# stoneMo/DeepAVFusion

Hardware: AMD Instinct MI355X
Metric: AV-pairs/sec, DeepAVFusion ViT-B pre-training step (224px + 10s audio, image mask 0.75) (higher is better)
Workload: dtype bf16; 1 GPU; AVMAE(DeepAVFusion base) fwd+bwd+allreduce+AdamW, B=64/GPU, 224x224 RGB + (128,640) log-mel, masks 0.75/0.8, fusion attn_ratio 0.25 mlp_ratio 1.0; global_batch=64, parallelism=dp1, graph=True

## Files before the change

### deepavfusion_amd/csrc/gemm_tn_gang.h

```cpp
#pragma once

__device__ __attribute__((aligned(256))) unsigned short g_tng_zeros[128];

struct TGDesc { int prob; int bnbk; };
struct TGHeader {
  int head[8];
  int q_start[9];
  int pad[15];
};
static_assert(sizeof(TGHeader) == 128, "TGHeader layout");

constexpr int TG_WCH = 28;
constexpr int TG_WIT = 72;
struct TGItem { int prob, desc_first, r0c0, nrnc; };
struct TGWrite {
  char* ws;
  int prob_first, prob_count, item_count, count_total, write_header;
  int q_start[9];
  TNParams prob[TG_WCH];
  TGItem item[TG_WIT];
};
static_assert(sizeof(TGWrite) <= 4096, "kernel argument block");

__global__ __launch_bounds__(64) void gemm_tn_gang_write_kernel(const TGWrite w) {
  TGHeader* hd = reinterpret_cast<TGHeader*>(w.ws);
  TNParams* probs = reinterpret_cast<TNParams*>(w.ws + sizeof(TGHeader));
  TGDesc* desc = reinterpret_cast<TGDesc*>(w.ws + sizeof(TGHeader) + (size_t)w.count_total * sizeof(TNParams));
  const int b = blockIdx.x, t = threadIdx.x;
  if (b < w.item_count) {
    const TGItem it = w.item[b];
    const int nr = it.nrnc >> 16, nc = it.nrnc & 0xffff, r0 = it.r0c0 >> 16, c0 = it.r0c0 & 0xffff;
    for (int i = t; i < nr * nc; i += 64) desc[it.desc_first + i] = TGDesc{it.prob, ((r0 + i / nc) << 16) | (c0 + i % nc)};
    return;
  }
  const int* src = reinterpret_cast<const int*>(w.prob);
  int* dst = reinterpret_cast<int*>(probs + w.prob_first);
  for (int i = t; i < w.prob_count * (int)(sizeof(TNParams) / 4); i += 64) dst[i] = src[i];
  if (w.write_header) {
    if (t < 8) hd->head[t] = 0;
    if (t < 9) hd->q_start[t] = w.q_start[t];
  }
}

__device__ __forceinline__ uint32_t tng_magic(int rpb) { return rpb > 1 ? (uint32_t)(0x100000000ull / (uint32_t)rpb) : rpb == 1 ? 0xffffffffu : 0u; }
__device__ __forceinline__ long tng_row(int m, const RowMap& r, uint32_t magic) {
  if (r.rpb <= 0) return (long)m;
  int q = (int)__umulhi((uint32_t)m, magic);
  int rem = m - q * r.rpb;
  if (rem >= r.rpb) { rem -= r.rpb; ++q; }
  return (long)q * r.bs + r.off + rem;
}

template <int V> struct TGI { static constexpr int value = V; };
template <int OFF>
__device__ __forceinline__ bf16x8 tng_tr(uint32_t base) {
  static_assert(OFF >= 0 && OFF + 1024 < 65536, "ds offset field");
  union { s16x4 h2[2]; bf16x8 v; } u;
  asm volatile("ds_read_b64_tr_b16 %0, %2 offset:%3\n\tds_read_b64_tr_b16 %1, %2 offset:%4"
               : "=&v"(u.h2[0]), "=&v"(u.h2[1]) : "v"(base), "i"(OFF), "i"(OFF + 1024));
  return u.v;
}

__device__ __forceinline__ void tng_tile(const TNParams& p, const int bn, const int bk, const int dbg) {
  extern __shared__ __attribute__((aligned(16))) char smem[];
  const int tid = threadIdx.x, lane = tid & 63;
  const int wave = __builtin_amdgcn_readfirstlane(tid >> 6);
  const int wr = wave >> 2, wc = wave & 3;
  const int n0 = bn << 8, k0 = bk << 8;
  const int nk = (p.Mc + 63) >> 6;
  const int kend = (nk + 1) & ~1;
  const uint32_t amagic = tng_magic(p.amap.rpb), bmagic = tng_magic(p.bmap.rpb);

  int a_col[2], b_col[2], krow[2];
#pragma unroll
  for (int ee = 0; ee < 2; ++ee) krow[ee] = (wave * 2 + ee) * 4 + (lane >> 4);
#pragma unroll
  for (int h = 0; h < 2; ++h) {
    const int c16 = lane & 15;
    const int g = (c16 >> 1) ^ (2 * ((lane >> 4) & 3));
    int ac = n0 + h * 128 + g * 16 + (c16 & 1) * 8; ac = ac < p.N ? ac : p.N - 8;
    int bc = k0 + h * 128 + g * 16 + (c16 & 1) * 8; bc = bc < p.K ? bc : p.K - 8;
    a_col[h] = ac; b_col[h] = bc;
  }
  auto issue = [&](bool isA, int h, int d, int kt) {
    char* slot = smem + (isA ? 0 : NT256_BREG) + d * 32768 + h * NT256_HT + wave * 2048;
    const bool pad = kt >= nk;
    const int ktc = pad ? nk - 1 : kt;
#pragma unroll
    for (int ee = 0; ee < 2; ++ee) {
      const int m0 = ktc * 64 + krow[ee];
      const int m = m0 < p.Mc ? m0 : p.Mc - 1;
      const bf16_t* src;
      if (isA) src = (pad || m0 >= p.Mc) ? reinterpret_cast<const bf16_t*>(g_tng_zeros) + (lane & 15) * 8 : p.A + tng_row(m, p.amap, amagic) * p.lda + a_col[h];
      else src = p.B + tng_row(m, p.bmap, bmagic) * p.ldb + b_col[h];
      __builtin_amdgcn_global_load_lds(GLB_PTR(void, src), LDS_PTR(void, slot + ee * 1024), 16, 0, 0);
    }
// ... 95 lines not shown
      TNG_G0(0, 1, t + 1) TNG_G0(1, 1, t + 1) TNG_G0(2, 1, t + 1) TNG_G0(3, 1, t + 1)
    }
#undef TNG_G0
  } else {
#define TNG_G1(I, D, T)                                                              \
    {                                                                                \
      if ((I) == 0) { read_a(TGI<(D) * 32768>{}); read_b(b0, TGI<(D) * 32768>{}); }                              \
      if ((I) == 1) read_b(b1, TGI<(D) * 32768 + 16384>{});                                              \
      if ((I) == 2) read_a(TGI<(D) * 32768 + 16384>{});                                                  \
      TNG_SB;                                                                        \
      issue_for(I, D, T);                                                            \
      asm volatile("s_waitcnt lgkmcnt(0)" ::: "memory");                             \
      TNG_SB;                                                                        \
      if ((I) == 0) bias_acc(0);                                                     \
      if ((I) == 2) bias_acc(1);                                                     \
      __builtin_amdgcn_s_setprio(1);                                                 \
      mfmas((I) >> 1, ((I) == 1 || (I) == 2) ? 1 : 0);                              \
      __builtin_amdgcn_s_setprio(0);                                                 \
      TNG_SB;                                                                        \
      wait_vmcnt<6>();                                                               \
      TNG_SB;                                                                        \
      __builtin_amdgcn_s_barrier();                                                  \
      TNG_SB;                                                                        \
    }
    for (int t = 0; t < kend; t += 2) {
      TNG_G1(0, 0, t) TNG_G1(1, 0, t) TNG_G1(2, 0, t) TNG_G1(3, 0, t)
      TNG_G1(0, 1, t + 1) TNG_G1(1, 1, t + 1) TNG_G1(2, 1, t + 1) TNG_G1(3, 1, t + 1)
    }
#undef TNG_G1
  }
#undef TNG_SB
  asm volatile("s_waitcnt vmcnt(0)" ::: "memory");
  __builtin_amdgcn_s_barrier();

  if (dbg & 2) return;
  typedef __attribute__((address_space(1))) f32x4 gf4_t;
  __attribute__((address_space(1))) float* const Cg = (__attribute__((address_space(1))) float*)p.C;
#pragma unroll
  for (int qm = 0; qm < 2; ++qm)
#pragma unroll
    for (int rf = 0; rf < 2; ++rf) {
      const int n = n0 + qm * 128 + wr * 64 + rf * 32 + (lane & 31);
      const long rowoff = (long)(n < p.N ? n : p.N - 1) * p.ldc;
      f32x4 v[2][4];
#pragma unroll
      for (int qn = 0; qn < 2; ++qn)
#pragma unroll
        for (int g = 0; g < 4; ++g) {
          const f32x16& q = acc[qm][qn][rf];
          v[qn][g] = f32x4{q[4 * g + 0], q[4 * g + 1], q[4 * g + 2], q[4 * g + 3]};
        }
      if (p.beta) {
        f32x4 old[2][4];
#pragma unroll
        for (int qn = 0; qn < 2; ++qn)
#pragma unroll
          for (int g = 0; g < 4; ++g) {
            const int k = k0 + qn * 128 + wc * 32 + 8 * g + 4 * hi;
            old[qn][g] = *(const gf4_t*)(Cg + rowoff + (k < p.K ? k : p.K - 4));
          }
#pragma unroll
        for (int qn = 0; qn < 2; ++qn)
#pragma unroll
          for (int g = 0; g < 4; ++g) v[qn][g] += old[qn][g];
      }
#pragma unroll
      for (int qn = 0; qn < 2; ++qn)
#pragma unroll
        for (int g = 0; g < 4; ++g) {
          const int k = k0 + qn * 128 + wc * 32 + 8 * g + 4 * hi;
          if (n < p.N && k < p.K) *(gf4_t*)(Cg + rowoff + k) = v[qn][g];
        }
    }
  if (do_bias) {
#pragma unroll
    for (int qm = 0; qm < 2; ++qm)
#pragma unroll
      for (int rf = 0; rf < 2; ++rf) {
        const float tot = accb[qm][rf] + __shfl_xor(accb[qm][rf], 32, 64);
        const int n = n0 + qm * 128 + wr * 64 + rf * 32 + (lane & 31);
        if (hi == 0 && n < p.N) unsafeAtomicAdd(p.bias_grad + n, tot);
      }
  }
}

constexpr size_t TNG_LDS = NT256_LDS + 16;

__global__ __launch_bounds__(512) void gemm_tn_gang_kernel(char* __restrict__ ws, const int count, const int dbg) {
  extern __shared__ __attribute__((aligned(16))) char smem[];
  TGHeader* hd = reinterpret_cast<TGHeader*>(ws);
  const int* probs = reinterpret_cast<const int*>(ws + sizeof(TGHeader));
  const TGDesc* desc = reinterpret_cast<const TGDesc*>(ws + sizeof(TGHeader) + (size_t)count * sizeof(TNParams));
  volatile __attribute__((address_space(3))) int* slot = (volatile __attribute__((address_space(3))) int*)(smem + NT256_LDS);
  int xcd;
  asm volatile("s_getreg_b32 %0, hwreg(HW_REG_XCC_ID)" : "=s"(xcd));
  xcd &= 7;
  if (dbg & 8) xcd = blockIdx.x & 7;
  if (dbg & 16) xcd = (blockIdx.x >> 5) & 7;
  for (int a = 0; a < 8; ++a) {
    const int q = (xcd + a) & 7;
    const int qs = hd->q_start[q], qn = hd->q_start[q + 1] - qs;
    while (true) {
      if (threadIdx.x == 0) {
        const int t = __hip_atomic_load(&hd->head[q], __ATOMIC_RELAXED, __HIP_MEMORY_SCOPE_AGENT) >= qn
                          ? qn : __hip_atomic_fetch_add(&hd->head[q], 1, __ATOMIC_RELAXED, __HIP_MEMORY_SCOPE_AGENT);
        *slot = t;
      }
      __syncthreads();
      const int t = __builtin_amdgcn_readfirstlane(*slot);
      __syncthreads();
      if (t >= qn) break;
      const TGDesc d = desc[qs + t];
      const int pi = __builtin_amdgcn_readfirstlane(d.prob), bnbk = __builtin_amdgcn_readfirstlane(d.bnbk);
      union { TNParams p; int w[sizeof(TNParams) / 4]; } u;
#pragma unroll
      for (int i = 0; i < (int)(sizeof(TNParams) / 4); ++i) u.w[i] = __builtin_amdgcn_readfirstlane(probs[pi * (int)(sizeof(TNParams) / 4) + i]);
      tng_tile(u.p, bnbk >> 16, bnbk & 0xffff, dbg);
    }
  }
}
```

### deepavfusion_amd/_lib.py

```python
from __future__ import annotations

import ctypes as C
import os

import torch

_HERE = os.path.dirname(os.path.abspath(__file__))
LIB_PATH = os.path.join(_HERE, 'libdavfusion_hip.so')

_p, _i, _l, _f, _sz = C.c_void_p, C.c_int, C.c_long, C.c_float, C.c_size_t

ABI_VERSION = 9

SIGNATURES = {
    'dav_abi_version': [],
    'dav_build_flags': [],
    'dav_last_error_string': [],
    'dav_tune': [_i, _i],
    'dav_gemm_nt_bf16': [_p, _p, _i, _i, _i, _i, _i, _p, _p, _i, _p, _i, _p, _i, _p, _p, _p, _i, _i, _p, _p, _i, _i, _i, _f, _i, _p],
    'dav_gemm_nt_ln_bf16': [_p, _p, _i, _i, _i, _i, _i, _p, _p, _i, _p, _i, _p, _i, _p, _p, _p, _i, _i, _p, _p, _i, _i, _i, _f, _i, _p, _p],
    'dav_ln_fold_grouped': [_p, _i, _p],
    'dav_rowstats_cast': [_p, _l, _i, _i, _i, _p, _p, _p],
    'dav_layernorm_bwd_twin': [_p, _l, _p, _i, _p, _l, _p, _i, _i, _i, _f, _p, _p, _p, _p,
                               _p, _l, _i, _p, _l, _p, _l,
                               _p, _l, _i, _p, _l, _p, _l,
                               _p, _p, _p, _p, _sz, _p],
    'dav_nt_issue_log': [_i, _p, _i],
    'dav_nt_tune_set': [_p, _i],
    'dav_gemm_tn_bf16': [_p, _p, _i, _i, _i, _i, _i, _p, _p, _p, _i, _i, _p, _i, _p],
    'dav_gemm_tn_grouped_bf16': [_p, _i, _p],
    'dav_gemm_tn_gang_workspace_bytes': [_p, _i],
    'dav_gemm_tn_gang_bf16': [_p, _i, _p, _sz, _p],
    'dav_attn_fwd': [_p, _p, _p, _p, _p, _i, _i, _i, _i, _i, _i, _l, _i, _l, _i, _l, _i, _l, _i, _f, _p],
    'dav_attn_bwd': [_p] * 10 + [_i] * 6 + [_l, _i] * 8 + [_f, _p],
    'dav_attn_bwd_part': [_p] * 10 + [_i] * 6 + [_l, _i] * 8 + [_f, _i, _p],
    'dav_add_cast': [_p, _p, _p, _p, _l, _p],
    'dav_attn_bwd_ctx': [_p] * 10 + [_i] * 6 + [_l, _i] * 8 + [_f, _i, _i, _p],
    'dav_attn_bias_fwd': [_p, _p, _p, _p, _p, _i, _i, _i, _i, _i, _i, _l, _i, _l, _i, _l, _i, _l, _i, _f, _p, _i, _i, _p],
    'dav_attn_bias_bwd': [_p] * 10 + [_i] * 6 + [_l, _i] * 8 + [_f, _p, _i, _i, _p, _i, _p],
    'dav_attn_drop_fwd': [_p, _p, _p, _p, _p, _i, _i, _i, _i, _i, _i, _l, _i, _l, _i, _l, _i, _l, _i, _f, _p, _i, _f, _p],
    'dav_attn_drop_bwd': [_p] * 10 + [_i] * 6 + [_l, _i] * 8 + [_f, _p, _i, _f, _i, _i, _p],
    'dav_window_unfold': [_p, _i, _p, _i, _i, _i, _i, _i, _i, _f, _p, _i, _p],
    'dav_window_fold': [_p, _p, _p, _i, _i, _i, _i, _i, _i, _f, _p, _p],
    'dav_relpos_bias_build': [_p, _p, _p, _i, _i, _i, _i, _i, _f, _p, _p],
    'dav_relpos_bias_bwd': [_p, _p, _i, _i, _i, _i, _i, _i, _p, _p],
    'dav_layernorm_fwd': [_p, _l, _i, _p, _l, _i, _i, _i, _p, _p, _f, _p, _p, _p, _p, _p],
    'dav_layernorm_bwd': [_p, _l, _i, _p, _l, _i, _i, _i, _p, _p, _p, _p, _p,
                          _p, _l, _i, _p, _l, _p, _l,
                          _p, _l, _i, _p, _l, _p, _l,
                          _p, _p, _p, _sz, _p],
    'dav_layernorm_bwd_workspace_bytes': [_i, _i],
    'dav_layernorm_bwd_reduce_grouped': [_p, _i, _p],
    'dav_mask_build': [_p, _i, _i, _i, _p, _p, _p, _p, _p, _p],
    'dav_patch_gather': [_p, _i, _i, _i, _i, _p, _i, _p, _p],
    'dav_patch_gather3d': [_p, _i, _i, _i, _i, _i, _i, _p, _i, _p, _p],
    'dav_unshuffle_fwd': [_p, _p, _p, _p, _i, _i, _i, _i, _p, _l, _i, _p],
    'dav_rows_gather_cast': [_p, _l, _i, _p, _i, _i, _i, _p, _p],
    'dav_rows_axpy': [_p, _p, _p, _i, _i, _i, _p, _p],
    'dav_rows_scale_cast': [_p, _p, _i, _i, _i, _p, _p],
    'dav_dropout_rows': [_p, _i, _p, _p, _f, _p, _i, _i, _i, _p, _i, _p],
    'dav_unshuffle_bwd_reduce': [_p, _l, _i, _p, _i, _i, _i, _i, _p, _p, _p],
    'dav_patch_mse_fwd': [_p, _p, _p, _i, _i, _i, _i, _i, _p, _p, _p, _p, _p, _p],
    'dav_patch_mse_bwd': [_p, _p, _p, _p, _p, _p, _p, _i, _i, _i, _i, _p, _p],
    'dav_pair_expand': [_p, _p, _i, _i, _i, _i, _p, _p],
    'dav_pair_reduce': [_p, _i, _i, _i, _i, _p, _p, _p],
# ... 121 lines not shown
```

### deepavfusion_amd/csrc/gemm.hip

```cpp
#include <algorithm>
#include <array>
#include <atomic>
#include <cstdlib>
#include <map>
#include <mutex>
#include <vector>

#include "common.h"
#include "dav_kernels.h"

namespace {

struct RowMap {
  int rpb, bs, off;
};
__device__ __forceinline__ long map_row(int m, const RowMap& r) {
  return r.rpb > 0 ? (long)(m / r.rpb) * r.bs + r.off + (m % r.rpb) : (long)m;
}

struct NTParams {
  const bf16_t* A; const bf16_t* B;
  int M, N, K, lda, ldb;
  RowMap amap;
  const float* bias;
// ... 2039 lines not shown
    total_tiles += (long)((q.N + 127) / 128) * ((q.K + 127) / 128);
  }
  int first = 0;
  for (int i = 0; i < count; ++i) {
    const DavTnProblem& q = probs[i];
    TNParams& p = g.prob[i];
    p.A = (const bf16_t*)q.A; p.B = (const bf16_t*)q.B; p.Mc = q.Mc; p.N = q.N; p.K = q.K; p.lda = q.lda; p.ldb = q.ldb;
    p.amap = RowMap{q.a_rowmap[0], q.a_rowmap[1], q.a_rowmap[2]};
    p.bmap = RowMap{q.b_rowmap[0], q.b_rowmap[1], q.b_rowmap[2]};
    static const int tn_debug = getenv("DAV_TN_DEBUG") ? atoi(getenv("DAV_TN_DEBUG")) & 6 : 0;
    p.C = q.C; p.ldc = q.ldc; p.beta = (q.flags & 1) ? 0 : 1; p.bias_grad = q.bias_grad; p.debug_plain_store = tn_debug;
    const int tiles = ((q.N + 127) / 128) * ((q.K + 127) / 128), steps = q.Mc >> 6;
    int splits = (int)((1024 + total_tiles - 1) / total_tiles);
    const int max_splits = steps / 8 > 0 ? steps / 8 : 1;
    if (splits > max_splits) splits = max_splits;
    if (q.flags & 1) splits = 1;
    p.splits = splits;
    g.first_block[i] = first;
    first += tiles * splits;
  }
  g.first_block[count] = first;
  g.count = count | TN_XCD_RUNS;
  const TNGroup gl = g;
  DAV_LAUNCH((gemm_tn_grouped_kernel<128, 4, 2>), dim3(first), dim3(512), (size_t)2 * 2 * 64 * 128 * 2, stream, gl);
  return dav_launch_status();
}

extern "C" int dav_gemm_tn_grouped_bf16(const DavTnProblem* probs, int count, hipStream_t stream) {
  if (!probs) return DAV_ERR_SHAPE;
  return tn_grouped_impl(probs, count, stream);
}

namespace {
struct TGPlanItem { int prob, r0, c0, nr, nc; long weight; int queue, first; };
long tn_gang_plan(const DavTnProblem* probs, int count, std::vector<TGPlanItem>& items, int q_start[9]) {
  items.clear();
  for (int i = 0; i < count; ++i) {
    const DavTnProblem& q = probs[i];
    const int tn = (q.N + 255) / 256, tk = (q.K + 255) / 256;
    int nr = tn, nc = tk;
    while (nr * nc > 32) { if (nr >= nc) nr = (nr + 1) / 2; else nc = (nc + 1) / 2; }
    for (int r0 = 0; r0 < tn; r0 += nr)
      for (int c0 = 0; c0 < tk; c0 += nc) {
        const int r = std::min(nr, tn - r0), c = std::min(nc, tk - c0);
        items.push_back(TGPlanItem{i, r0, c0, r, c, (long)r * c * ((q.Mc + 127) / 128), 0, 0});
      }
  }
  std::vector<int> order(items.size());
  for (size_t i = 0; i < order.size(); ++i) order[i] = (int)i;
  std::stable_sort(order.begin(), order.end(), [&](int a, int b) { return probs[items[a].prob].Mc > probs[items[b].prob].Mc; });
  long load[8] = {0, 0, 0, 0, 0, 0, 0, 0};
  int tiles_q[8] = {0, 0, 0, 0, 0, 0, 0, 0};
  for (int oi : order) {
    int best = 0;
    for (int q = 1; q < 8; ++q) if (load[q] < load[best]) best = q;
    items[oi].queue = best; items[oi].first = tiles_q[best];
    load[best] += items[oi].weight; tiles_q[best] += items[oi].nr * items[oi].nc;
  }
  q_start[0] = 0;
  for (int q = 0; q < 8; ++q) q_start[q + 1] = q_start[q] + tiles_q[q];
  return q_start[8];
}
int tn_gang_check(const DavTnProblem* probs, int count) {
  if (count <= 0 || count > 4096) return DAV_ERR_SHAPE;
  for (int i = 0; i < count; ++i) {
    const DavTnProblem& q = probs[i];
    if (q.Mc <= 0 || q.N <= 0 || q.K <= 0 || (q.N & 7) || (q.K & 7) || (q.lda & 7) || (q.ldb & 7)) return DAV_ERR_SHAPE;
    if (q.N > (32767 << 8) || q.K > (32767 << 8) || (q.flags & ~1)) return DAV_ERR_SHAPE;
    if (((uintptr_t)q.A | (uintptr_t)q.B | (uintptr_t)q.C) & 15 || (q.ldc & 3)) return DAV_ERR_ALIGN;
  }
  return DAV_OK;
}
}

extern "C" size_t dav_gemm_tn_gang_workspace_bytes(const DavTnProblem* probs, int count) {
  if (!probs || tn_gang_check(probs, count) != DAV_OK) return 0;
  long tiles = 0;
  for (int i = 0; i < count; ++i) tiles += (long)((probs[i].N + 255) / 256) * ((probs[i].K + 255) / 256);
  return sizeof(TGHeader) + (size_t)count * sizeof(TNParams) + (size_t)tiles * sizeof(TGDesc);
}

extern "C" int dav_gemm_tn_gang_bf16(const DavTnProblem* probs, int count, void* workspace, size_t workspace_bytes, hipStream_t stream) {
  if (!probs || !workspace) return DAV_ERR_SHAPE;
  const int chk = tn_gang_check(probs, count);
  if (chk != DAV_OK) return chk;
  if ((uintptr_t)workspace & 15) return DAV_ERR_ALIGN;
  if (workspace_bytes < dav_gemm_tn_gang_workspace_bytes(probs, count)) return DAV_ERR_WORKSPACE;
  std::vector<TGPlanItem> items;
  int q_start[9];
  tn_gang_plan(probs, count, items, q_start);
#ifdef DAV_EXPERIMENTAL
  static const int dbg = getenv("DAV_TN_GANG_DEBUG") ? atoi(getenv("DAV_TN_GANG_DEBUG")) & 30 : 0;
#else
  static const int dbg = getenv("DAV_TN_GANG_DEBUG") ? atoi(getenv("DAV_TN_GANG_DEBUG")) & 24 : 0;
#endif
  bool header = true;
  std::vector<std::vector<const TGPlanItem*>> by_prob(count);
  for (const TGPlanItem& it : items) by_prob[it.prob].push_back(&it);
  TGWrite w;
  auto reset = [&](int first) {
    w.ws = (char*)workspace; w.prob_first = first; w.prob_count = 0; w.item_count = 0; w.count_total = count; w.write_header = 0;
    for (int q = 0; q < 9; ++q) w.q_start[q] = q_start[q];
  };
  auto flush = [&]() {
    if (!w.prob_count && !w.item_count && !header) return;
    w.write_header = header ? 1 : 0; header = false;
    const TGWrite wl = w;
    DAV_LAUNCH(gemm_tn_gang_write_kernel, dim3(wl.item_count + 1), dim3(64), 0, stream, wl);
  };
  reset(0);
  for (int i = 0; i < count; ++i) {
    if (w.prob_count == TG_WCH) { flush(); reset(i); }
    const DavTnProblem& q = probs[i];
    TNParams& p = w.prob[w.prob_count++];
    p.A = (const bf16_t*)q.A; p.B = (const bf16_t*)q.B; p.Mc = q.Mc; p.N = q.N; p.K = q.K; p.lda = q.lda; p.ldb = q.ldb;
    p.amap = RowMap{q.a_rowmap[0], q.a_rowmap[1], q.a_rowmap[2]};
    p.bmap = RowMap{q.b_rowmap[0], q.b_rowmap[1], q.b_rowmap[2]};
    p.C = q.C; p.ldc = q.ldc; p.beta = (q.flags & 1) ? 0 : 1; p.bias_grad = q.bias_grad; p.debug_plain_store = 0; p.splits = 1;
    for (const TGPlanItem* it : by_prob[i]) {
      if (w.item_count == TG_WIT) { flush(); reset(i + 1); }
      w.item[w.item_count++] = TGItem{i, q_start[it->queue] + it->first, (it->r0 << 16) | it->c0, (it->nr << 16) | it->nc};
    }
  }
  flush();
  static std::mutex dev_mu;
  static int dev_cus[64] = {0};
  int n_wg = 256;
  {
    int dev = 0;
    if (hipGetDevice(&dev) != hipSuccess || dev < 0 || dev >= 64) return DAV_ERR_HIP;
    std::lock_guard<std::mutex> lk(dev_mu);
    if (!dev_cus[dev]) {
      if (hipFuncSetAttribute((const void*)gemm_tn_gang_kernel, hipFuncAttributeMaxDynamicSharedMemorySize, 160 * 1024) != hipSuccess) return DAV_ERR_HIP;
      int cus = 256;
      (void)hipDeviceGetAttribute(&cus, hipDeviceAttributeMultiprocessorCount, dev);
      dev_cus[dev] = cus > 0 ? cus : 256;
    }
    n_wg = dev_cus[dev];
  }
  const long tiles = q_start[8];
  const int grid = (int)std::min<long>(n_wg, tiles);
  DAV_LAUNCH(gemm_tn_gang_kernel, dim3(grid), dim3(512), TNG_LDS, stream, (char*)workspace, count, dbg);
  return dav_launch_status();
}

extern "C" int dav_gemm_tn_bf16(const void* A, const void* B, int Mc, int N, int K, int lda, int ldb,
                                const int* a_rowmap, const int* b_rowmap, float* C, int ldc, int beta,
                                float* bias_grad, int variant, hipStream_t stream) {
  if (Mc <= 0 || N <= 0 || K <= 0 || (N & 7) || (K & 7) || (lda & 7) || (ldb & 7)) return DAV_ERR_SHAPE;
  if (((uintptr_t)A | (uintptr_t)B) & 15) return DAV_ERR_ALIGN;
  TNParams p;
  p.A = (const bf16_t*)A; p.B = (const bf16_t*)B; p.Mc = Mc; p.N = N; p.K = K; p.lda = lda; p.ldb = ldb;
  p.amap = mk(a_rowmap); p.bmap = mk(b_rowmap); p.C = C; p.ldc = ldc; p.beta = beta; p.bias_grad = bias_grad;
  p.debug_plain_store = (variant >> 8) & 1;
  variant &= ~256;
  const int steps = (Mc + 63) / 64;
  const int cfg = variant >> 4;
  if (!(variant & 15) && (Mc & 63) == 0 && (beta || cfg) && !(ldc & 3) && !((uintptr_t)C & 15)) {
    const int t128 = ((N + 127) / 128) * ((K + 127) / 128), t64 = ((N + 63) / 64) * ((K + 63) / 64);
    const bool big = cfg ? cfg == 1 : (Mc >= 20000 && t128 >= 48);
    const int tiles = big ? t128 : t64;
    int splits = beta ? (768 + tiles - 1) / tiles : 1;
    const int max_splits = steps / 6 > 0 ? steps / 6 : 1;
    if (splits > max_splits) splits = max_splits;
    p.splits = splits;
    if (big) launch_tn2<128, 2, 4>(p, tiles, stream);
    else launch_tn2<64, 2, 2>(p, tiles, stream);
    return dav_launch_status();
  }
  const int tiles = ((N + 127) / 128) * ((K + 127) / 128);
  int splits = 1;
  if (beta) {
    splits = (1024 + tiles - 1) / tiles;
    if (splits > steps) splits = steps;
    if (splits > 64) splits = 64;
// ... 9 lines not shown
```

### include/dav_kernels.h

```cpp
#ifndef DAV_KERNELS_H_
#define DAV_KERNELS_H_

#include <stddef.h>
#include <stdint.h>

#ifdef __HIPCC__
#include <hip/hip_runtime.h>
#else
typedef struct ihipStream_t* hipStream_t;
#endif

#ifdef __cplusplus
extern "C" {
#endif

#define DAV_ABI_VERSION 9
int dav_abi_version(void);
int dav_build_flags(void);
const char* dav_last_error_string(void);
int dav_tune(int knob, int value);

int dav_gemm_nt_bf16(const void* A, const void* B, int M, int N, int K, int lda, int ldb, const int* a_rowmap,
                     const float* bias, int act, const void* aux, int ldaux, const float* res, int ldres,
                     const int* res_rowmap, const int* res_rows, void* C, int ldc, int c_is_bf16, const int* c_rowmap,
                     void* C2, int ldc2, int c2_mode, int beta, float alpha, int variant, hipStream_t stream);

typedef struct DavNtLn {
  const float* stats; const float* stats2; const void* A2; const float* ln_c; float eps; int a_r0, a_r1;
  float* stats_out; void* twin_out; int ld_twin;
} DavNtLn;
int dav_gemm_nt_ln_bf16(const void* A, const void* B, int M, int N, int K, int lda, int ldb, const int* a_rowmap,
                        const float* bias, int act, const void* aux, int ldaux, const float* res, int ldres,
                        const int* res_rowmap, const int* res_rows, void* C, int ldc, int c_is_bf16, const int* c_rowmap,
                        void* C2, int ldc2, int c2_mode, int beta, float alpha, int variant, const DavNtLn* ln, hipStream_t stream);

int dav_nt_issue_log(int enable, int* out, int capacity);

int dav_nt_tune_set(const int* blob, int n_ints);

int dav_gemm_tn_bf16(const void* A, const void* B, int Mc, int N, int K, int lda, int ldb, const int* a_rowmap,
                     const int* b_rowmap, float* C, int ldc, int beta, float* bias_grad, int variant, hipStream_t stream);

typedef struct DavTnProblem {
  const void* A; const void* B;
  float* C; float* bias_grad;
  int Mc, N, K, lda, ldb, ldc;
  int a_rowmap[3], b_rowmap[3];
  int flags;
} DavTnProblem;
int dav_gemm_tn_grouped_bf16(const DavTnProblem* problems, int count, hipStream_t stream);

size_t dav_gemm_tn_gang_workspace_bytes(const DavTnProblem* problems, int count);
int dav_gemm_tn_gang_bf16(const DavTnProblem* problems, int count, void* workspace, size_t workspace_bytes, hipStream_t stream);

int dav_attn_fwd(const void* Q, const void* K, const void* V, void* O, float* LSE, int B, int H, int Nq, int Nk, int dqk,
                 int dv, long q_bs, int q_rs, long k_bs, int k_rs, long v_bs, int v_rs, long o_bs, int o_rs, float scale,
                 hipStream_t stream);
int dav_attn_bwd(const void* Q, const void* K, const void* V, const void* O, const void* dO, const float* LSE, float* Delta,
                 void* dQ, void* dK, void* dV, int B, int H, int Nq, int Nk, int dqk, int dv, long q_bs, int q_rs, long k_bs,
                 int k_rs, long v_bs, int v_rs, long o_bs, int o_rs, long do_bs, int do_rs, long dq_bs, int dq_rs, long dk_bs,
                 int dk_rs, long dv_bs, int dv_rs, float scale, hipStream_t stream);
int dav_attn_bwd_part(const void* Q, const void* K, const void* V, const void* O, const void* dO, const float* LSE, float* Delta,
                 void* dQ, void* dK, void* dV, int B, int H, int Nq, int Nk, int dqk, int dv, long q_bs, int q_rs, long k_bs,
                 int k_rs, long v_bs, int v_rs, long o_bs, int o_rs, long do_bs, int do_rs, long dq_bs, int dq_rs, long dk_bs,
                 int dk_rs, long dv_bs, int dv_rs, float scale, int part, hipStream_t stream);

int dav_attn_bwd_ctx(const void* Q, const void* K, const void* V, const void* O, const void* dO, const float* LSE, float* Delta,
                 void* dQ, void* dK, void* dV, int B, int H, int Nq, int Nk, int dqk, int dv, long q_bs, int q_rs, long k_bs,
                 int k_rs, long v_bs, int v_rs, long o_bs, int o_rs, long do_bs, int do_rs, long dq_bs, int dq_rs, long dk_bs,
                 int dk_rs, long dv_bs, int dv_rs, float scale, int dq_ctx_rows, int part, hipStream_t stream);

int dav_attn_bias_fwd(const void* Q, const void* K, const void* V, void* O, float* LSE, int B, int H, int Nq, int Nk, int dqk,
                      int dv, long q_bs, int q_rs, long k_bs, int k_rs, long v_bs, int v_rs, long o_bs, int o_rs, float scale,
                      const float* bias, int bias_nb, int bias_ld, hipStream_t stream);
int dav_attn_bias_bwd(const void* Q, const void* K, const void* V, const void* O, const void* dO, const float* LSE, float* Delta,
                      void* dQ, void* dK, void* dV, int B, int H, int Nq, int Nk, int dqk, int dv, long q_bs, int q_rs, long k_bs,
                      int k_rs, long v_bs, int v_rs, long o_bs, int o_rs, long do_bs, int do_rs, long dq_bs, int dq_rs, long dk_bs,
                      int dk_rs, long dv_bs, int dv_rs, float scale, const float* bias, int bias_nb, int bias_ld, float* dS,
                      int part, hipStream_t stream);

int dav_attn_drop_fwd(const void* Q, const void* K, const void* V, void* O, float* LSE, int B, int H, int Nq, int Nk, int dqk,
                      int dv, long q_bs, int q_rs, long k_bs, int k_rs, long v_bs, int v_rs, long o_bs, int o_rs, float scale,
                      const void* keep, int keep_ld, float keep_scale, hipStream_t stream);
int dav_attn_drop_bwd(const void* Q, const void* K, const void* V, const void* O, const void* dO, const float* LSE, float* Delta,
                      void* dQ, void* dK, void* dV, int B, int H, int Nq, int Nk, int dqk, int dv, long q_bs, int q_rs, long k_bs,
                      int k_rs, long v_bs, int v_rs, long o_bs, int o_rs, long do_bs, int do_rs, long dq_bs, int dq_rs, long dk_bs,
// ... 138 lines not shown
```

Before: 2571 AV-pairs/s.

## Prefetch next gang tile descriptor before epilogue via LDS staging

The persistent TN gang GEMM kernel now claims its next work item from the atomic queue and stages that problem's TNParams and tile id into LDS before the current tile's epilogue runs, not after it finishes. Threads load the params in parallel into shared memory rather than each lane doing serial scalar global loads. This hides the queue-atomic and descriptor-load latency behind the epilogue stores. In exchange it uses a little more LDS and adds an extra __syncthreads per claimed tile.

After: 2578 AV-pairs/s (median of 6 runs). No clear change (+0.3%).

```diff
diff --git a/deepavfusion_amd/csrc/gemm_tn_gang.h b/deepavfusion_amd/csrc/gemm_tn_gang.h
--- a/deepavfusion_amd/csrc/gemm_tn_gang.h
+++ b/deepavfusion_amd/csrc/gemm_tn_gang.h
@@ -61,7 +61,8 @@
   return u.v;
 }
 
-__device__ __forceinline__ void tng_tile(const TNParams& p, const int bn, const int bk, const int dbg) {
+template <typename F>
+__device__ __forceinline__ void tng_tile(const TNParams& p, const int bn, const int bk, const int dbg, F&& before_epilogue) {
   extern __shared__ __attribute__((aligned(16))) char smem[];
   const int tid = threadIdx.x, lane = tid & 63;
   const int wave = __builtin_amdgcn_readfirstlane(tid >> 6);
@@ -223,6 +224,7 @@
 #undef TNG_SB
   asm volatile("s_waitcnt vmcnt(0)" ::: "memory");
   __builtin_amdgcn_s_barrier();
+  before_epilogue();
 
   if (dbg & 2) return;
   typedef __attribute__((address_space(1))) f32x4 gf4_t;
@@ -275,7 +277,9 @@
   }
 }
 
-constexpr size_t TNG_LDS = NT256_LDS + 16;
+constexpr int TNG_PW = (int)(sizeof(TNParams) / 4);
+static_assert(TNG_PW % 4 == 0, "staged TNParams are read as 16-byte words");
+constexpr size_t TNG_LDS = NT256_LDS + 16 + (TNG_PW + 1) * 4;
 
 __global__ __launch_bounds__(512) void gemm_tn_gang_kernel(char* __restrict__ ws, const int count, const int dbg) {
   extern __shared__ __attribute__((aligned(16))) char smem[];
@@ -283,30 +287,47 @@
   const int* probs = reinterpret_cast<const int*>(ws + sizeof(TGHeader));
   const TGDesc* desc = reinterpret_cast<const TGDesc*>(ws + sizeof(TGHeader) + (size_t)count * sizeof(TNParams));
   volatile __attribute__((address_space(3))) int* slot = (volatile __attribute__((address_space(3))) int*)(smem + NT256_LDS);
+  __attribute__((address_space(3))) int* const next = (__attribute__((address_space(3))) int*)(smem + NT256_LDS + 16);
   int xcd;
   asm volatile("s_getreg_b32 %0, hwreg(HW_REG_XCC_ID)" : "=s"(xcd));
   xcd &= 7;
   if (dbg & 8) xcd = blockIdx.x & 7;
   if (dbg & 16) xcd = (blockIdx.x >> 5) & 7;
-  for (int a = 0; a < 8; ++a) {
-    const int q = (xcd + a) & 7;
-    const int qs = hd->q_start[q], qn = hd->q_start[q + 1] - qs;
-    while (true) {
+  int a = 0;
+  auto draw = [&]() -> bool {
+#pragma nounroll
+    for (; a < 8; ++a) {
+      const int q = (xcd + a) & 7;
+      const int qs = hd->q_start[q], qn = hd->q_start[q + 1] - qs;
       if (threadIdx.x == 0) {
-        const int t = __hip_atomic_load(&hd->head[q], __ATOMIC_RELAXED, __HIP_MEMORY_SCOPE_AGENT) >= qn
-                          ? qn : __hip_atomic_fetch_add(&hd->head[q], 1, __ATOMIC_RELAXED, __HIP_MEMORY_SCOPE_AGENT);
-        *slot = t;
+        *slot = __hip_atomic_load(&hd->head[q], __ATOMIC_RELAXED, __HIP_MEMORY_SCOPE_AGENT) >= qn
+                    ? qn : __hip_atomic_fetch_add(&hd->head[q], 1, __ATOMIC_RELAXED, __HIP_MEMORY_SCOPE_AGENT);
       }
       __syncthreads();
       const int t = __builtin_amdgcn_readfirstlane(*slot);
       __syncthreads();
-      if (t >= qn) break;
-      const TGDesc d = desc[qs + t];
-      const int pi = __builtin_amdgcn_readfirstlane(d.prob), bnbk = __builtin_amdgcn_readfirstlane(d.bnbk);
-      union { TNParams p; int w[sizeof(TNParams) / 4]; } u;
-#pragma unroll
-      for (int i = 0; i < (int)(sizeof(TNParams) / 4); ++i) u.w[i] = __builtin_amdgcn_readfirstlane(probs[pi * (int)(sizeof(TNParams) / 4) + i]);
-      tng_tile(u.p, bnbk >> 16, bnbk & 0xffff, dbg);
-    }
-  }
-}
+      if (t < qn) {
+        if (threadIdx.x <= TNG_PW) {
+          const TGDesc d = desc[qs + t];
+          next[threadIdx.x] = threadIdx.x < TNG_PW ? probs[d.prob * TNG_PW + threadIdx.x] : d.bnbk;
+        }
+        __syncthreads();
+        return true;
+      }
+    }
+    return false;
+  };
+  bool more = draw();
+  while (more) {
+    union { TNParams p; int w[TNG_PW]; } u;
+    typedef __attribute__((ext_vector_type(4))) int i32x4;
+#pragma unroll
+    for (int i = 0; i < TNG_PW / 4; ++i) {
+      const i32x4 v = reinterpret_cast<__attribute__((address_space(3))) const i32x4*>(next)[i];
+#pragma unroll
+      for (int j = 0; j < 4; ++j) u.w[4 * i + j] = __builtin_amdgcn_readfirstlane(v[j]);
+    }
+    const int bnbk = __builtin_amdgcn_readfirstlane(next[TNG_PW]);
+    tng_tile(u.p, bnbk >> 16, bnbk & 0xffff, dbg, [&]() { more = draw(); });
+  }
+}
```

## Pack grouped TN gang GEMM tiles into length-matched rounds with load-ordered stealing

Applied to the files above, without the earlier changes.

Replaces the per-XCD queue planner for the grouped weight-gradient (TN) gang GEMM. Tiles are now packed into 32-tile rounds grouped by similar M length, and rounds are balanced across the 8 queues with greedy assignment plus swap refinement. A simple makespan model picks between this and the old ring plan. Work stealing now visits victim queues in order of heaviest load instead of a fixed ring. It also adds an opt-in timestamp recording path (a templated kernel variant) and a plan-query API for profiling, at the cost of more host-side planning work per launch.

New measurement: 2579 AV-pairs/s before, 2595 AV-pairs/s after (median of 6 runs). No clear change (+0.7%).

```diff
diff --git a/deepavfusion_amd/_lib.py b/deepavfusion_amd/_lib.py
--- a/deepavfusion_amd/_lib.py
+++ b/deepavfusion_amd/_lib.py
@@ -31,6 +31,8 @@
     'dav_gemm_tn_grouped_bf16': [_p, _i, _p],
     'dav_gemm_tn_gang_workspace_bytes': [_p, _i],
     'dav_gemm_tn_gang_bf16': [_p, _i, _p, _sz, _p],
+    'dav_gemm_tn_gang_plan': [_p, _i, _p, _i, _p, _p],
+    'dav_gemm_tn_gang_record': [_p, _sz],
     'dav_attn_fwd': [_p, _p, _p, _p, _p, _i, _i, _i, _i, _i, _i, _l, _i, _l, _i, _l, _i, _l, _i, _f, _p],
     'dav_attn_bwd': [_p] * 10 + [_i] * 6 + [_l, _i] * 8 + [_f, _p],
     'dav_attn_bwd_part': [_p] * 10 + [_i] * 6 + [_l, _i] * 8 + [_f, _i, _p],
diff --git a/deepavfusion_amd/csrc/gemm.hip b/deepavfusion_amd/csrc/gemm.hip
--- a/deepavfusion_amd/csrc/gemm.hip
+++ b/deepavfusion_amd/csrc/gemm.hip
@@ -2095,19 +2095,131 @@
 }
 
 namespace {
-struct TGPlanItem { int prob, r0, c0, nr, nc; long weight; int queue, first; };
-long tn_gang_plan(const DavTnProblem* probs, int count, std::vector<TGPlanItem>& items, int q_start[9]) {
+struct TGPlanItem { int prob, r0, c0, nr, nc; int len, round; int queue, first; };
+struct TGRound { int len, tiles, queue; long cost; bool mixed; std::vector<int> items; };
+inline int tn_gang_len(int Mc) { return (((Mc + 63) >> 6) + 1) & ~1; }
+long tn_gang_plan(const DavTnProblem* probs, int count, std::vector<TGPlanItem>& items, std::vector<TGRound>& rounds, int q_start[9], int victims[8]) {
+  items.clear(); rounds.clear();
+  std::vector<int> order(count);
+  for (int i = 0; i < count; ++i) order[i] = i;
+  std::stable_sort(order.begin(), order.end(), [&](int a, int b) { return tn_gang_len(probs[a].Mc) > tn_gang_len(probs[b].Mc); });
+  std::vector<int> open;
+  auto put = [&](int item, int ri) {
+    TGRound& r = rounds[ri];
+    TGPlanItem& it = items[item];
+    it.round = ri;
+    r.items.push_back(item); r.tiles += it.nr * it.nc; r.mixed = r.mixed || it.len != r.len;
+    if (r.tiles >= 32) open.erase(std::find(open.begin(), open.end(), ri));
+  };
+  auto new_round = [&](int len) {
+    rounds.push_back(TGRound{len, 0, 0, len, false, {}});
+    open.push_back((int)rounds.size() - 1);
+    return (int)rounds.size() - 1;
+  };
+  auto find_round = [&](int tiles, int len) {
+    for (int ri : open) if (rounds[ri].len == len && rounds[ri].tiles + tiles <= 32) return ri;
+    for (size_t k = open.size(); k-- > 0;) if (rounds[open[k]].tiles + tiles <= 32) return open[k];
+    return -1;
+  };
+  for (int o = 0; o < count;) {
+    int oe = o;
+    const int len = tn_gang_len(probs[order[o]].Mc);
+    while (oe < count && tn_gang_len(probs[order[oe]].Mc) == len) ++oe;
+    std::vector<int> whole;
+    for (int k = o; k < oe; ++k) {
+      const int i = order[k];
+      const int tn = (probs[i].N + 255) / 256, tk = (probs[i].K + 255) / 256;
+      if (tn * tk <= 32) { whole.push_back((int)items.size()); items.push_back(TGPlanItem{i, 0, 0, tn, tk, len, 0, 0, 0}); continue; }
+      if (std::min(tn, tk) <= 16) {
+        const bool cols = tk >= tn;
+        const int s = cols ? tn : tk, n = cols ? tk : tn, full = 32 / s;
+        for (int at = 0; at < n;) {
+          int take = std::min(full, n - at);
+          if (n - at - take == 1 && take > 2) --take;
+          whole.push_back((int)items.size());
+          items.push_back(cols ? TGPlanItem{i, 0, at, tn, take, len, 0, 0, 0} : TGPlanItem{i, at, 0, take, tk, len, 0, 0, 0});
+          at += take;
+        }
+        continue;
+      }
+      int nr = tn, nc = tk;
+      while (nr * nc > 32) { if (nr >= nc) nr = (nr + 1) / 2; else nc = (nc + 1) / 2; }
+      for (int r0 = 0; r0 < tn; r0 += nr)
+        for (int c0 = 0; c0 < tk; c0 += nc) {
+          whole.push_back((int)items.size());
+          items.push_back(TGPlanItem{i, r0, c0, std::min(nr, tn - r0), std::min(nc, tk - c0), len, 0, 0, 0});
+        }
+    }
+    std::stable_sort(whole.begin(), whole.end(), [&](int a, int b) { return items[a].nr * items[a].nc > items[b].nr * items[b].nc; });
+    for (int w : whole) {
+      int ri = find_round(items[w].nr * items[w].nc, len);
+      if (ri < 0) ri = new_round(len);
+      put(w, ri);
+    }
+    o = oe;
+  }
+  const int nr = (int)rounds.size();
+  std::vector<int> ro(nr);
+  for (int i = 0; i < nr; ++i) ro[i] = i;
+  std::stable_sort(ro.begin(), ro.end(), [&](int a, int b) { return rounds[a].cost > rounds[b].cost; });
+  long load[8] = {0, 0, 0, 0, 0, 0, 0, 0};
+  for (int ri : ro) {
+    int best = 0;
+    for (int q = 1; q < 8; ++q) if (load[q] < load[best]) best = q;
+    rounds[ri].queue = best; load[best] += rounds[ri].cost;
+  }
+  for (int pass = 0; pass < 64 && nr <= 1024; ++pass) {
+    int hi = 0;
+    for (int q = 1; q < 8; ++q) if (load[q] > load[hi]) hi = q;
+    long best_max = load[hi]; int ba = -1, bb = -1;
+    for (int a = 0; a < nr; ++a) {
+      if (rounds[a].queue != hi) continue;
+      for (int q = 0; q < 8; ++q) {
+        if (q == hi) continue;
+        const long m = std::max(load[hi] - rounds[a].cost, load[q] + rounds[a].cost);
+        if (m < best_max) { best_max = m; ba = a; bb = -1 - q; }
+      }
+      for (int b = 0; b < nr; ++b) {
+        const int q = rounds[b].queue;
+        if (q == hi || rounds[b].cost >= rounds[a].cost) continue;
+        const long d = rounds[a].cost - rounds[b].cost;
+        const long m = std::max(load[hi] - d, load[q] + d);
+        if (m < best_max) { best_max = m; ba = a; bb = b; }
+      }
+    }
+    if (ba < 0) break;
+    if (bb < 0) { const int q = -1 - bb; load[hi] -= rounds[ba].cost; load[q] += rounds[ba].cost; rounds[ba].queue = q; }
+    else { const int q = rounds[bb].queue; const long d = rounds[ba].cost - rounds[bb].cost; load[hi] -= d; load[q] += d; rounds[ba].queue = q; rounds[bb].queue = hi; }
+  }
+  std::stable_sort(ro.begin(), ro.end(), [&](int a, int b) { return rounds[a].len > rounds[b].len; });
+  int tiles_q[8] = {0, 0, 0, 0, 0, 0, 0, 0};
+  for (int ri : ro)
+    for (int it : rounds[ri].items) {
+      const int q = rounds[ri].queue;
+      items[it].queue = q; items[it].first = tiles_q[q];
+      tiles_q[q] += items[it].nr * items[it].nc;
+    }
+  q_start[0] = 0;
+  for (int q = 0; q < 8; ++q) q_start[q + 1] = q_start[q] + tiles_q[q];
+  for (int x = 0; x < 8; ++x) {
+    int qs[8], n = 0;
+    for (int q = 0; q < 8; ++q) if (q != x) qs[n++] = q;
+    std::stable_sort(qs, qs + 7, [&](int a, int b) { return load[a] > load[b]; });
+    int v = x;
+    for (int a = 0; a < 7; ++a) v |= qs[a] << (4 * (a + 1));
+    victims[x] = v;
+  }
+  return q_start[8];
+}
+long tn_gang_plan_ring(const DavTnProblem* probs, int count, std::vector<TGPlanItem>& items, int q_start[9], int victims[8]) {
   items.clear();
   for (int i = 0; i < count; ++i) {
-    const DavTnProblem& q = probs[i];
-    const int tn = (q.N + 255) / 256, tk = (q.K + 255) / 256;
+    const int tn = (probs[i].N + 255) / 256, tk = (probs[i].K + 255) / 256;
     int nr = tn, nc = tk;
     while (nr * nc > 32) { if (nr >= nc) nr = (nr + 1) / 2; else nc = (nc + 1) / 2; }
     for (int r0 = 0; r0 < tn; r0 += nr)
-      for (int c0 = 0; c0 < tk; c0 += nc) {
-        const int r = std::min(nr, tn - r0), c = std::min(nc, tk - c0);
-        items.push_back(TGPlanItem{i, r0, c0, r, c, (long)r * c * ((q.Mc + 127) / 128), 0, 0});
-      }
+      for (int c0 = 0; c0 < tk; c0 += nc)
+        items.push_back(TGPlanItem{i, r0, c0, std::min(nr, tn - r0), std::min(nc, tk - c0), tn_gang_len(probs[i].Mc), (int)items.size(), 0, 0});
   }
   std::vector<int> order(items.size());
   for (size_t i = 0; i < order.size(); ++i) order[i] = (int)i;
@@ -2118,12 +2230,50 @@
     int best = 0;
     for (int q = 1; q < 8; ++q) if (load[q] < load[best]) best = q;
     items[oi].queue = best; items[oi].first = tiles_q[best];
-    load[best] += items[oi].weight; tiles_q[best] += items[oi].nr * items[oi].nc;
+    load[best] += (long)items[oi].nr * items[oi].nc * ((probs[items[oi].prob].Mc + 127) / 128); tiles_q[best] += items[oi].nr * items[oi].nc;
   }
   q_start[0] = 0;
   for (int q = 0; q < 8; ++q) q_start[q + 1] = q_start[q] + tiles_q[q];
+  for (int x = 0; x < 8; ++x) {
+    victims[x] = 0;
+    for (int a = 0; a < 8; ++a) victims[x] |= ((x + a) & 7) << (4 * a);
+  }
   return q_start[8];
 }
+long tn_gang_makespan(const std::vector<TGPlanItem>& items) {
+  std::vector<std::pair<int, int>> tk[8];
+  for (size_t i = 0; i < items.size(); ++i) tk[items[i].queue].push_back({items[i].first, (int)i});
+  long worst = 0;
+  for (int q = 0; q < 8; ++q) {
+    std::sort(tk[q].begin(), tk[q].end());
+    std::vector<long> cu(32, 0);
+    auto later = [](long a, long b) { return a > b; };
+    for (auto& t : tk[q])
+      for (int k = 0; k < items[t.second].nr * items[t.second].nc; ++k) {
+        std::pop_heap(cu.begin(), cu.end(), later);
+        cu.back() += items[t.second].len;
+        worst = std::max(worst, cu.back());
+        std::push_heap(cu.begin(), cu.end(), later);
+      }
+  }
+  return worst;
+}
+long tn_gang_plan_for(const DavTnProblem* probs, int count, int which, std::vector<TGPlanItem>& items, int q_start[9], int victims[8]) {
+  std::vector<TGRound> rounds;
+  if (which & 32) return tn_gang_plan_ring(probs, count, items, q_start, victims);
+  if (which & 64) return tn_gang_plan(probs, count, items, rounds, q_start, victims);
+  std::vector<TGPlanItem> ring;
+  int rq[9], rv[8];
+  const long tiles = tn_gang_plan_ring(probs, count, ring, rq, rv);
+  tn_gang_plan(probs, count, items, rounds, q_start, victims);
+  if (50 * tn_gang_makespan(items) < 49 * tn_gang_makespan(ring)) return tiles;
+  items.swap(ring);
+  for (int q = 0; q < 9; ++q) q_start[q] = rq[q];
+  for (int q = 0; q < 8; ++q) victims[q] = rv[q];
+  return tiles;
+}
+std::atomic<int*> tn_gang_rec{nullptr};
+std::atomic<int> tn_gang_rec_cap{0};
 int tn_gang_check(const DavTnProblem* probs, int count) {
   if (count <= 0 || count > 4096) return DAV_ERR_SHAPE;
   for (int i = 0; i < count; ++i) {
@@ -2143,6 +2293,36 @@
   return sizeof(TGHeader) + (size_t)count * sizeof(TNParams) + (size_t)tiles * sizeof(TGDesc);
 }
 
+extern "C" int dav_gemm_tn_gang_plan(const DavTnProblem* probs, int count, int* gangs, int capacity_ints, int* q_start_out, int* victims_out) {
+  if (!probs || count <= 0 || count > 4096) return DAV_ERR_SHAPE;
+  for (int i = 0; i < count; ++i)
+    if (probs[i].Mc <= 0 || probs[i].N <= 0 || probs[i].K <= 0 || probs[i].N > (32767 << 8) || probs[i].K > (32767 << 8)) return DAV_ERR_SHAPE;
+  std::vector<TGPlanItem> items;
+  int q_start[9], victims[8];
+  tn_gang_plan_for(probs, count, 0, items, q_start, victims);
+  const int n = (int)items.size();
+  if (q_start_out) for (int q = 0; q < 9; ++q) q_start_out[q] = q_start[q];
+  if (victims_out) for (int q = 0; q < 8; ++q) victims_out[q] = victims[q];
+  if (!gangs) return n;
+  if (capacity_ints < 8 * n) return DAV_ERR_WORKSPACE;
+  for (int i = 0; i < n; ++i) {
+    const TGPlanItem& it = items[i];
+    const int g[8] = {it.queue, it.first, it.prob, it.r0, it.c0, it.nr, it.nc, it.round};
+    for (int k = 0; k < 8; ++k) gangs[8 * i + k] = g[k];
+  }
+  return n;
+}
+
+extern "C" int dav_gemm_tn_gang_record(void* buf, size_t bytes) {
+  if (!buf) return DAV_ERR_SHAPE;
+  if ((uintptr_t)buf & 15) return DAV_ERR_ALIGN;
+  if (bytes == 0) { tn_gang_rec.store(nullptr); tn_gang_rec_cap.store(0); return DAV_OK; }
+  if (bytes < 64 + sizeof(TGRecord)) return DAV_ERR_WORKSPACE;
+  tn_gang_rec_cap.store((int)std::min<size_t>((bytes - 64) / sizeof(TGRecord), 1u << 30));
+  tn_gang_rec.store((int*)buf);
+  return DAV_OK;
+}
+
 extern "C" int dav_gemm_tn_gang_bf16(const DavTnProblem* probs, int count, void* workspace, size_t workspace_bytes, hipStream_t stream) {
   if (!probs || !workspace) return DAV_ERR_SHAPE;
   const int chk = tn_gang_check(probs, count);
@@ -2150,13 +2330,13 @@
   if ((uintptr_t)workspace & 15) return DAV_ERR_ALIGN;
   if (workspace_bytes < dav_gemm_tn_gang_workspace_bytes(probs, count)) return DAV_ERR_WORKSPACE;
   std::vector<TGPlanItem> items;
-  int q_start[9];
-  tn_gang_plan(probs, count, items, q_start);
+  int q_start[9], victims[8];
 #ifdef DAV_EXPERIMENTAL
-  static const int dbg = getenv("DAV_TN_GANG_DEBUG") ? atoi(getenv("DAV_TN_GANG_DEBUG")) & 30 : 0;
+  static const int dbg = getenv("DAV_TN_GANG_DEBUG") ? atoi(getenv("DAV_TN_GANG_DEBUG")) & 126 : 0;
 #else
-  static const int dbg = getenv("DAV_TN_GANG_DEBUG") ? atoi(getenv("DAV_TN_GANG_DEBUG")) & 24 : 0;
+  static const int dbg = getenv("DAV_TN_GANG_DEBUG") ? atoi(getenv("DAV_TN_GANG_DEBUG")) & 120 : 0;
 #endif
+  tn_gang_plan_for(probs, count, dbg, items, q_start, victims);
   bool header = true;
   std::vector<std::vector<const TGPlanItem*>> by_prob(count);
   for (const TGPlanItem& it : items) by_prob[it.prob].push_back(&it);
@@ -2164,6 +2344,7 @@
   auto reset = [&](int first) {
     w.ws = (char*)workspace; w.prob_first = first; w.prob_count = 0; w.item_count = 0; w.count_total = count; w.write_header = 0;
     for (int q = 0; q < 9; ++q) w.q_start[q] = q_start[q];
+    for (int q = 0; q < 8; ++q) w.victims[q] = victims[q];
   };
   auto flush = [&]() {
     if (!w.prob_count && !w.item_count && !header) return;
@@ -2194,7 +2375,8 @@
     if (hipGetDevice(&dev) != hipSuccess || dev < 0 || dev >= 64) return DAV_ERR_HIP;
     std::lock_guard<std::mutex> lk(dev_mu);
     if (!dev_cus[dev]) {
-      if (hipFuncSetAttribute((const void*)gemm_tn_gang_kernel, hipFuncAttributeMaxDynamicSharedMemorySize, 160 * 1024) != hipSuccess) return DAV_ERR_HIP;
+      if (hipFuncSetAttribute((const void*)gemm_tn_gang_kernel<false>, hipFuncAttributeMaxDynamicSharedMemorySize, 160 * 1024) != hipSuccess) return DAV_ERR_HIP;
+      if (hipFuncSetAttribute((const void*)gemm_tn_gang_kernel<true>, hipFuncAttributeMaxDynamicSharedMemorySize, 160 * 1024) != hipSuccess) return DAV_ERR_HIP;
       int cus = 256;
       (void)hipDeviceGetAttribute(&cus, hipDeviceAttributeMultiprocessorCount, dev);
       dev_cus[dev] = cus > 0 ? cus : 256;
@@ -2203,7 +2385,10 @@
   }
   const long tiles = q_start[8];
   const int grid = (int)std::min<long>(n_wg, tiles);
-  DAV_LAUNCH(gemm_tn_gang_kernel, dim3(grid), dim3(512), TNG_LDS, stream, (char*)workspace, count, dbg);
+  int* const rec = tn_gang_rec.load();
+  const int rec_cap = tn_gang_rec_cap.load();
+  if (rec) DAV_LAUNCH(gemm_tn_gang_kernel<true>, dim3(grid), dim3(512), TNG_LDS, stream, (char*)workspace, count, dbg, rec, rec_cap);
+  else DAV_LAUNCH(gemm_tn_gang_kernel<false>, dim3(grid), dim3(512), TNG_LDS, stream, (char*)workspace, count, dbg, (int*)nullptr, 0);
   return dav_launch_status();
 }
 
diff --git a/deepavfusion_amd/csrc/gemm_tn_gang.h b/deepavfusion_amd/csrc/gemm_tn_gang.h
--- a/deepavfusion_amd/csrc/gemm_tn_gang.h
+++ b/deepavfusion_amd/csrc/gemm_tn_gang.h
@@ -6,7 +6,8 @@
 struct TGHeader {
   int head[8];
   int q_start[9];
-  int pad[15];
+  int victims[8];
+  int pad[7];
 };
 static_assert(sizeof(TGHeader) == 128, "TGHeader layout");
 
@@ -17,6 +18,7 @@
   char* ws;
   int prob_first, prob_count, item_count, count_total, write_header;
   int q_start[9];
+  int victims[8];
   TNParams prob[TG_WCH];
   TGItem item[TG_WIT];
 };
@@ -39,6 +41,7 @@
   if (w.write_header) {
     if (t < 8) hd->head[t] = 0;
     if (t < 9) hd->q_start[t] = w.q_start[t];
+    if (t < 8) hd->victims[t] = w.victims[t];
   }
 }
 
@@ -61,7 +64,8 @@
   return u.v;
 }
 
-__device__ __forceinline__ void tng_tile(const TNParams& p, const int bn, const int bk, const int dbg) {
+template <bool REC>
+__device__ __forceinline__ void tng_tile(const TNParams& p, const int bn, const int bk, const int dbg, uint64_t& t_loop_end) {
   extern __shared__ __attribute__((aligned(16))) char smem[];
   const int tid = threadIdx.x, lane = tid & 63;
   const int wave = __builtin_amdgcn_readfirstlane(tid >> 6);
@@ -223,6 +227,7 @@
 #undef TNG_SB
   asm volatile("s_waitcnt vmcnt(0)" ::: "memory");
   __builtin_amdgcn_s_barrier();
+  if (REC) t_loop_end = __builtin_amdgcn_s_memrealtime();
 
   if (dbg & 2) return;
   typedef __attribute__((address_space(1))) f32x4 gf4_t;
@@ -277,7 +282,11 @@
 
 constexpr size_t TNG_LDS = NT256_LDS + 16;
 
-__global__ __launch_bounds__(512) void gemm_tn_gang_kernel(char* __restrict__ ws, const int count, const int dbg) {
+struct TGRecord { int where, prob, bnbk, ticket; uint32_t t_start, t_loop_end, t_end, t_hi; };
+static_assert(sizeof(TGRecord) == 32, "TGRecord layout");
+
+template <bool REC>
+__global__ __launch_bounds__(512) void gemm_tn_gang_kernel(char* __restrict__ ws, const int count, const int dbg, int* __restrict__ rec, const int rec_cap) {
   extern __shared__ __attribute__((aligned(16))) char smem[];
   TGHeader* hd = reinterpret_cast<TGHeader*>(ws);
   const int* probs = reinterpret_cast<const int*>(ws + sizeof(TGHeader));
@@ -286,17 +295,29 @@
   int xcd;
   asm volatile("s_getreg_b32 %0, hwreg(HW_REG_XCC_ID)" : "=s"(xcd));
   xcd &= 7;
+  const int xcc = xcd;
   if (dbg & 8) xcd = blockIdx.x & 7;
   if (dbg & 16) xcd = (blockIdx.x >> 5) & 7;
+  const int order = hd->victims[xcd];
+  uint64_t t0 = 0, t1 = 0, t2 = 0;
+  int r_where = -1, r_pi = 0, r_bnbk = 0, r_ticket = 0;
   for (int a = 0; a < 8; ++a) {
-    const int q = (xcd + a) & 7;
+    const int q = (order >> (4 * a)) & 7;
     const int qs = hd->q_start[q], qn = hd->q_start[q + 1] - qs;
     while (true) {
       if (threadIdx.x == 0) {
+        if (REC && r_where >= 0) {
+          const int i = __hip_atomic_fetch_add(rec, 1, __ATOMIC_RELAXED, __HIP_MEMORY_SCOPE_AGENT);
+          if (i < rec_cap) {
+            TGRecord r{r_where, r_pi, r_bnbk, r_ticket, (uint32_t)t0, (uint32_t)t1, (uint32_t)t2, (uint32_t)(t0 >> 32)};
+            reinterpret_cast<TGRecord*>(rec + 16)[i] = r;
+          }
+        }
         const int t = __hip_atomic_load(&hd->head[q], __ATOMIC_RELAXED, __HIP_MEMORY_SCOPE_AGENT) >= qn
                           ? qn : __hip_atomic_fetch_add(&hd->head[q], 1, __ATOMIC_RELAXED, __HIP_MEMORY_SCOPE_AGENT);
         *slot = t;
       }
+      if (REC) r_where = -1;
       __syncthreads();
       const int t = __builtin_amdgcn_readfirstlane(*slot);
       __syncthreads();
@@ -306,7 +327,12 @@
       union { TNParams p; int w[sizeof(TNParams) / 4]; } u;
 #pragma unroll
       for (int i = 0; i < (int)(sizeof(TNParams) / 4); ++i) u.w[i] = __builtin_amdgcn_readfirstlane(probs[pi * (int)(sizeof(TNParams) / 4) + i]);
-      tng_tile(u.p, bnbk >> 16, bnbk & 0xffff, dbg);
-    }
-  }
-}
+      if (REC) t0 = __builtin_amdgcn_s_memrealtime();
+      tng_tile<REC>(u.p, bnbk >> 16, bnbk & 0xffff, dbg, t1);
+      if (REC) {
+        t2 = __builtin_amdgcn_s_memrealtime();
+        r_where = xcc | (q << 8) | ((int)blockIdx.x << 16); r_pi = pi; r_bnbk = bnbk; r_ticket = qs + t;
+      }
+    }
+  }
+}
diff --git a/include/dav_kernels.h b/include/dav_kernels.h
--- a/include/dav_kernels.h
+++ b/include/dav_kernels.h
@@ -52,6 +52,8 @@
 
 size_t dav_gemm_tn_gang_workspace_bytes(const DavTnProblem* problems, int count);
 int dav_gemm_tn_gang_bf16(const DavTnProblem* problems, int count, void* workspace, size_t workspace_bytes, hipStream_t stream);
+int dav_gemm_tn_gang_plan(const DavTnProblem* problems, int count, int* gangs, int capacity_ints, int* q_start, int* victims);
+int dav_gemm_tn_gang_record(void* buf, size_t bytes);
 
 int dav_attn_fwd(const void* Q, const void* K, const void* V, void* O, float* LSE, int B, int H, int Nq, int Nk, int dqk,
                  int dv, long q_bs, int q_rs, long k_bs, int k_rs, long v_bs, int v_rs, long o_bs, int o_rs, float scale,
```
